# ZhangT-tech/MoCA-Video

Hardware: AMD Instinct MI355X
Metric: denoising UNet-steps/sec @16x320x512 fp16 (higher is better)
Workload: dtype f16

## Files before the change

include/moca_hip.h:

```cpp
#ifndef MOCA_HIP_H
#define MOCA_HIP_H

#include <stdint.h>

#ifdef __cplusplus
extern "C" {
#endif

#define MOCA_OK            0
#define MOCA_E_BADARG     -1
#define MOCA_E_LAUNCH     -2
#define MOCA_E_NODEVICE   -3
#define MOCA_E_GRAPH      -4

#define MOCA_A_LINEAR   0
#define MOCA_A_CONV3X3  1
#define MOCA_A_TCONV3   2

#define MOCA_EP_GEGLU   1
#define MOCA_EP_OUT_F32 2
#define MOCA_FORCE_SMALL_TILE 4
#define MOCA_EP_COLSUM 16
#define MOCA_EP_LN     32
#define MOCA_EP_GELU    8
// ... 44 lines not shown
    float       tattn_scale;
    const void* prefetch;
    int32_t     up_phase;
    int32_t     reserved4_;
    const void* a2;
    int32_t     lda2;
    int32_t     k1;
    int32_t     gstat_cpg;
    int32_t     gstat_coff;
    int32_t     wgroup_rows;
    int32_t     wgroup_stride;
} moca_gemm_params;

int moca_gemm_f16(const moca_gemm_params* p, void* stream);
int moca_gemm_colsum_rows(const moca_gemm_params* p);
int moca_gemm_ln_ok(const moca_gemm_params* p);
int moca_gemm_rowsum_cols(const moca_gemm_params* p);
int moca_gemm_lnfold_ok(const moca_gemm_params* p);
int moca_gemm_tattn_ok(const moca_gemm_params* p);
int moca_gemm_wgroup_ok(const moca_gemm_params* p);
int moca_gemm_cat_ok(const moca_gemm_params* p);
#define MOCA_ROUTE_SMALL64   1
#define MOCA_ROUTE_SMALL128  2
#define MOCA_ROUTE_GLDS128   3
#define MOCA_ROUTE_GLDS160   4
#define MOCA_ROUTE_G4        5
#define MOCA_ROUTE_W80       6
#define MOCA_ROUTE_W80W      7
#define MOCA_ROUTE_SQ256     8
#define MOCA_ROUTE_G4P       9
#define MOCA_ROUTE_SQP       10
#define MOCA_ROUTE_TATTN     11
#define MOCA_ROUTE_WS        12
int moca_gemm_route(const moca_gemm_params* p);
int moca_gemm_splitk_groupnorm_ok(const moca_gemm_params* p, int32_t HW, int32_t frames_per_stat);
int moca_gemm_splitk_groupnorm_f16(const moca_gemm_params* p, void* y, const float* gamma, const float* beta, int32_t HW,
                                   int32_t frames_per_stat, float eps, int32_t silu, int32_t write_x, void* stream);
int64_t moca_gemm_splitk_ws_bytes(int32_t M, int32_t N, int32_t splits);

int moca_groupnorm_nhwc_f16(const void* x, void* y, const float* gamma, const float* beta,
                            int32_t F, int32_t HW, int32_t C, int32_t frames_per_stat,
                            float eps, int32_t silu, float* ws, void* stream);
int64_t moca_groupnorm_ws_bytes(int32_t F, int32_t HW, int32_t C);
int moca_groupnorm_colsum_f16(const void* x, void* y, const float* gamma, const float* beta, const float* colsum,
                              int32_t tile_rows, int32_t F, int32_t HW, int32_t C, int32_t frames_per_stat,
                              float eps, int32_t silu, float* ws, void* stream);

int moca_groupnorm_fold_weights_f16(const void* w, const float* bias, const float* gamma, const float* beta, const int64_t* gstat,
                                    void* wg, float* bg, int32_t n_sg, int32_t N, int32_t K, int32_t ldw, int64_t count, float eps,
                                    void* stream);

int moca_groupnorm_gstat_f16(const void* x, void* y, const float* gamma, const float* beta, const int64_t* gstat,
                             int32_t F, int32_t HW, int32_t C, int32_t frames_per_stat,
                             float eps, int32_t silu, void* stream);
int moca_concat_channels_gstat_f16(const void* a, const void* b, void* out, int32_t F, int32_t HW, int32_t C1, int32_t C2,
                                   int32_t frames_per_stat, int64_t* gstat, void* stream);
int moca_groupnorm_gstat_cat_f16(const void* a, const void* b, void* y, const float* gamma, const float* beta,
                                 const int64_t* gstat_cat, const int64_t* gstat_b, int32_t Fb, int32_t F, int32_t HW, int32_t C1,
                                 int32_t C2, int32_t frames_per_stat, float eps, int32_t silu, void* stream);
int moca_gstat_accum_f16(const void* x, int32_t F, int32_t HW, int32_t C, int32_t frames_per_stat, int32_t cpg, int32_t coff,
                         int64_t* gstat, void* stream);
int moca_memset_zero(void* ptr, int64_t bytes, void* stream);

int moca_layernorm_f16(const void* x, void* y, const float* gamma, const float* beta,
                       int32_t M, int32_t C, float eps, void* stream);

// ... 117 lines not shown
int moca_base_ddim_step_f32(moca_fifo_state* state, float* x, const float* eps_c, const float* eps_u, const float* noise,
                            float* pred_x0, const float* coef, int32_t S, float cfg_scale, int32_t use_scale, int64_t n, void* stream);
int moca_mask_frame_sums_f32(const float* mask, float* sums, int32_t frames, int32_t HW, void* stream);

int moca_freq_mix_3d_f32(const float* x, const float* noise, const float* lpf, float* out,
                         int32_t C, int32_t T, int32_t H, int32_t W, float* ws, void* stream);
int64_t moca_freq_mix_ws_bytes(int32_t C, int32_t T, int32_t H, int32_t W);
int moca_freq_filter_f32(float* lpf, int32_t T, int32_t H, int32_t W, int32_t type, int32_t n,
                         double d_s, double d_t, void* stream);

int moca_graph_begin(void* stream);
int moca_graph_end(void* stream, void** graph_exec_out);
int moca_graph_launch(void* graph_exec, void* stream);
int moca_graph_destroy(void* graph_exec);
int moca_stream_create(void** stream_out);
int moca_stream_destroy(void* stream);
int moca_stream_sync(void* stream);
int moca_event_create(void** ev_out);
int moca_event_record(void* ev, void* stream);
int moca_event_elapsed_ms(void* ev_start, void* ev_stop, float* ms_out);
int moca_event_destroy(void* ev);

#define MOCA_TUNE_GEMM_W80   0
#define MOCA_TUNE_GEMM_G4    1
#define MOCA_TUNE_GEMM_SQ256 2
#define MOCA_TUNE_GEMM_WIDE  3
#define MOCA_TUNE_GN_SLAB    4
#define MOCA_TUNE_GEMM_G4P   5
#define MOCA_TUNE_GEMM_MF32  6
#define MOCA_TUNE_GEMM_SQP   7
#define MOCA_TUNE_SQP_WALK   8
#define MOCA_TUNE_SLAB_F16   9
#define MOCA_TUNE_GEMM_WS    10
#define MOCA_TUNE_COUNT      11
int moca_set_tuning(int32_t knob, int32_t value);
int moca_debug_clock_sampler(void* buf, int32_t blocks, int32_t nsamples, const int32_t* stop, void* stream);

int moca_device_info(char* name, int32_t len, int32_t* cu_count);
const char* moca_version(void);

#ifdef __cplusplus
}
#endif
#endif
```

moca_video_amd/csrc/common.h:

```cpp
#pragma once
#include <hip/hip_runtime.h>
#include <stdint.h>
#include "../../include/moca_hip.h"

typedef _Float16 half_t;
typedef _Float16 half2v __attribute__((ext_vector_type(2)));
typedef _Float16 half4v __attribute__((ext_vector_type(4)));
typedef _Float16 half8v __attribute__((ext_vector_type(8)));
typedef float    f32x4  __attribute__((ext_vector_type(4)));
typedef float    f32x16 __attribute__((ext_vector_type(16)));

#define MOCA_WAVE 64

#define MOCA_CHECK_LAUNCH()                                  \
    do {                                                     \
        hipError_t e__ = hipGetLastError();                  \
        if (e__ != hipSuccess) return MOCA_E_LAUNCH;         \
    } while (0)

static inline hipStream_t moca_stream(void* s) { return reinterpret_cast<hipStream_t>(s); }

int moca_tuning_get(int knob);

bool moca_gemm_ws_ok(const moca_gemm_params& p);
int moca_gemm_ws_launch(const moca_gemm_params& p, hipStream_t st);

__device__ __forceinline__ float moca_silu(float x) {
    return x * __builtin_amdgcn_rcpf(1.0f + __builtin_amdgcn_exp2f(x * -1.4426950408889634f));
}
typedef float f32x2 __attribute__((ext_vector_type(2)));
__device__ __forceinline__ float moca_erf(float x) {
    const float ax = fabsf(x);
    const float t = __builtin_amdgcn_rcpf(1.0f + 0.3275911f * ax);
    float y = 1.061405429f;
    y = y * t - 1.453152027f;
    y = y * t + 1.421413741f;
    y = y * t - 0.284496736f;
    y = y * t + 0.254829592f;
    y = 1.0f - y * t * __builtin_amdgcn_exp2f(ax * ax * -1.4426950408889634f);
    return copysignf(y, x);
}
__device__ __forceinline__ float moca_gelu(float x) { return 0.5f * x * (1.0f + moca_erf(x * 0.70710678118654752f)); }

__device__ __forceinline__ f32x2 moca_erf2(f32x2 x) {
    const f32x2 ax = {fabsf(x[0]), fabsf(x[1])};
    const f32x2 d = ax * 0.3275911f + 1.0f;
    const f32x2 t = {__builtin_amdgcn_rcpf(d[0]), __builtin_amdgcn_rcpf(d[1])};
    f32x2 y = t * 1.061405429f - 1.453152027f;
    y = y * t + 1.421413741f;
    y = y * t - 0.284496736f;
    y = y * t + 0.254829592f;
    const f32x2 a2 = ax * ax * -1.4426950408889634f;
    const f32x2 e = {__builtin_amdgcn_exp2f(a2[0]), __builtin_amdgcn_exp2f(a2[1])};
    y = 1.0f - y * t * e;
    return f32x2{copysignf(y[0], x[0]), copysignf(y[1], x[1])};
}
#ifdef MOCA_GELU_OLD
__device__ __forceinline__ f32x2 moca_geglu2(f32x2 v, f32x2 g) {
// ... 70 lines not shown
```

moca_video_amd/csrc/gemm.hip:

```cpp
#include "gemm_launch.h"

namespace {

template <int BN, int AMODE>
__global__ __launch_bounds__(256, 2) void gemm_f16_kernel(const moca_gemm_params p) {
    constexpr int NT = BN / 64;
    constexpr int B_SLOTS = BN / 32;
    constexpr int A_BYTES = BM * ROW_BYTES;
    constexpr int B_BYTES = BN * ROW_BYTES;

    extern __shared__ __attribute__((aligned(16))) char smem[];
    char* sA = smem;
    char* sB = smem + 2 * A_BYTES;

    const int tid = threadIdx.x, lane = tid & 63, wave = tid >> 6;
    const int wave_m = wave >> 1, wave_n = wave & 1;

    const int tiles_m = (p.M + BM - 1) / BM;
    const int tiles_n = p.N / BN;
    const int nblk = tiles_m * tiles_n * p.splits;
    int logical;
    remap_block<BN>(nblk, logical);
    const int split = logical % p.splits;
    const int tile = logical / p.splits;
// ... 389 lines not shown
            const int c0 = ccol[i] - g * cpg;
            half8v r;
#pragma unroll
            for (int j = 0; j < 8; ++j) {
                float a = (float)v[i][j] * s_sc[c0 + j] + s_sh[c0 + j];
                if (silu) a = moca_silu(a);
                r[j] = (half_t)a;
            }
            *reinterpret_cast<half8v*>(y + (int64_t)mrow[i] * N + ccol[i]) = r;
        }
}

template <int BN, int AMODE>
int launch_gemm(const moca_gemm_params& p, hipStream_t st) {
    const int tiles_m = (p.M + BM - 1) / BM, tiles_n = p.N / BN;
    const int nblk = tiles_m * tiles_n * p.splits;
    constexpr int lds_pipe = 2 * (BM + BN) * ROW_BYTES;
    constexpr int lds_epi = BM * BN * 4;
    constexpr int lds = lds_pipe > lds_epi ? lds_pipe : lds_epi;
    if (!dyn_lds_once<&gemm_f16_kernel<BN, AMODE>>(lds)) return MOCA_E_LAUNCH;
    hipLaunchKernelGGL((gemm_f16_kernel<BN, AMODE>), dim3(nblk), dim3(256), lds, st, p);
    MOCA_CHECK_LAUNCH();
    return MOCA_OK;
}
int launch_gemm_small(int bn, const moca_gemm_params& p, hipStream_t st) {
    if (bn == 128) return with_gather(p, [&](auto am, auto) { return launch_gemm<128, decltype(am)::value>(p, st); });
    return with_gather(p, [&](auto am, auto) { return launch_gemm<64, decltype(am)::value>(p, st); });
}

enum Route : int {
    R_NONE = 0,
    R_SMALL64 = MOCA_ROUTE_SMALL64, R_SMALL128 = MOCA_ROUTE_SMALL128, R_GLDS128 = MOCA_ROUTE_GLDS128, R_GLDS160 = MOCA_ROUTE_GLDS160,
    R_G4 = MOCA_ROUTE_G4, R_W80 = MOCA_ROUTE_W80, R_W80W = MOCA_ROUTE_W80W, R_SQ256 = MOCA_ROUTE_SQ256, R_G4P = MOCA_ROUTE_G4P,
    R_SQP = MOCA_ROUTE_SQP, R_TATTN = MOCA_ROUTE_TATTN, R_WS = MOCA_ROUTE_WS,
};

void normalise_splits(moca_gemm_params& p) {
    if (p.splits < 1) p.splits = 1;
    if (p.splits > (p.K + BK - 1) / BK) p.splits = (p.K + BK - 1) / BK;
    if (p.splits > 1) {
        const int nkt = (p.K + BK - 1) / BK, kts = (nkt + p.splits - 1) / p.splits;
        p.splits = (nkt + kts - 1) / kts;
    }
}

inline int64_t a_span_bytes(const moca_gemm_params& p) {
    if (p.a_mode == MOCA_A_LINEAR) return ((int64_t)p.M * p.lda + 64) * 2;
    if (p.a_mode == MOCA_A_CONV3X3) return ((int64_t)(p.M / (p.outH * p.outW)) * p.inH * p.inW * p.C + 64) * 2;
    return ((int64_t)p.M * p.C + 64) * 2;
}
inline bool buffer_addressable(const moca_gemm_params& p) {
    if (p.a2 && ((int64_t)p.M * p.lda2 + 64) * 2 >= (1ll << 31)) return false;
    return a_span_bytes(p) < (1ll << 31) && (int64_t)p.N * p.ldw * 2 < (1ll << 31);
}

bool persistent_ok(const moca_gemm_params& p, int BN, int blocks) {
    if (p.a_mode != MOCA_A_LINEAR || p.splits != 1 || p.N % BN || p.K % 64 || !buffer_addressable(p)) return false;
    if (p.flags & ~(MOCA_EP_GEGLU | MOCA_EP_LNFOLD)) return false;
    if ((p.flags & MOCA_EP_GEGLU) && (p.residual || p.rowadd)) return false;
    return ((p.M + 255) / 256) * (p.N / BN) >= blocks;
}

Route route_of(const moca_gemm_params& p) {
    if (p.flags & MOCA_EP_TATTN) return R_TATTN;
    const int ws_mode = moca_tuning_get(MOCA_TUNE_GEMM_WS);
    if (ws_mode && moca_gemm_ws_ok(p) && (ws_mode == 2 || p.residual || p.M >= (1 << 17))) return R_WS;
    if (!p.a2 && p.wgroup_rows <= 0) {
        const int sqp_mode = moca_tuning_get(MOCA_TUNE_GEMM_SQP), g4p_mode = moca_tuning_get(MOCA_TUNE_GEMM_G4P);
        if (sqp_mode && persistent_ok(p, 256, SQP_BLOCKS) && (sqp_mode == 2 || (p.flags & MOCA_EP_GEGLU))) return R_SQP;
        if (g4p_mode && persistent_ok(p, 128, G4P_BLOCKS) && (g4p_mode == 2 || (p.flags & MOCA_EP_GEGLU))) return R_G4P;
    }
    const int w80_mode = moca_tuning_get(MOCA_TUNE_GEMM_W80);
    const int tiles320 = ((p.M + 319) / 320) * (p.N / 160);
    if (w80_mode && p.N % 160 == 0 && !(p.flags & (MOCA_EP_GEGLU | MOCA_EP_OUT_F32 | MOCA_FORCE_SMALL_TILE)) && p.M > 160 &&
        (tiles320 * p.splits >= 200 || w80_mode == 2) && fast_gather(p) && buffer_addressable(p)) {
        if (p.flags & MOCA_EP_LN) return R_W80W;
        const int wide_mode = moca_tuning_get(MOCA_TUNE_GEMM_WIDE);
        if (wide_mode == 0 || p.N % 320) return R_W80;
        return (p.a_mode == MOCA_A_LINEAR || wide_mode == 2) ? R_W80W : R_W80;
    }
    const int g4_mode = moca_tuning_get(MOCA_TUNE_GEMM_G4);
    const bool use_g4 = !(p.flags & MOCA_EP_OUT_F32) &&
                        (g4_mode == 2 || (g4_mode == 1 && (p.flags & MOCA_EP_GEGLU) && p.K <= 640 && p.M < (1 << 17)));
    const int sq256_mode = moca_tuning_get(MOCA_TUNE_GEMM_SQ256);
    if (sq256_mode && p.a_mode == MOCA_A_LINEAR && p.N % 256 == 0 && p.N >= 2560 && p.M >= 512 && fast_gather(p) && buffer_addressable(p) &&
        !(p.flags & (MOCA_EP_OUT_F32 | MOCA_FORCE_SMALL_TILE)) && ((p.M + 255) / 256) * (p.N / 256) * p.splits >= 200 &&
        (sq256_mode == 2 || !use_g4)) return R_SQ256;
    const int big_bn = (p.N % 128 == 0) ? 128 : (p.N % 160 == 0 ? 160 : 0);
    if (big_bn != 0 && p.M > 128 && !(p.flags & MOCA_FORCE_SMALL_TILE)) {
        if (big_bn == 128) return use_g4 ? R_G4 : R_GLDS128;
        return R_GLDS160;
    }
    return p.N % 128 == 0 ? R_SMALL128 : R_SMALL64;
}

constexpr int CAN_SPLITK = 1 << 16, CAN_A2 = 1 << 17, CAN_WGROUP = 1 << 18, CAN_UP_PHASE = 1 << 19;
constexpr int EP_STATS = MOCA_EP_COLSUM | MOCA_EP_GSTAT;
struct RouteInfo { int tm, tn, can; };
RouteInfo route_info(Route r) {
    constexpr int GLDS = MOCA_EP_GEGLU | MOCA_EP_OUT_F32 | EP_STATS | MOCA_EP_ROWSUM | MOCA_EP_LNFOLD | CAN_SPLITK | CAN_UP_PHASE;
    constexpr int W80 = EP_STATS | MOCA_EP_ROWSUM | MOCA_EP_LNFOLD | CAN_SPLITK | CAN_UP_PHASE | CAN_A2 | CAN_WGROUP;
    switch (r) {
        case R_SMALL64: return {BM, 64, MOCA_EP_OUT_F32 | MOCA_EP_GELU | CAN_SPLITK};
        case R_SMALL128: return {BM, 128, MOCA_EP_GEGLU | MOCA_EP_OUT_F32 | MOCA_EP_GELU | CAN_SPLITK};
        case R_GLDS128: return {256, 128, GLDS};
        case R_GLDS160: return {256, 160, GLDS};
        case R_G4: return {256, 128, MOCA_EP_GEGLU | MOCA_EP_LNFOLD | CAN_SPLITK | CAN_UP_PHASE};
        case R_W80: return {320, 160, W80};
        case R_W80W: return {160, 320, W80 | MOCA_EP_LN};
        case R_SQ256: return {256, 256, MOCA_EP_GEGLU | MOCA_EP_LNFOLD | CAN_SPLITK};
        case R_G4P: return {256, 128, MOCA_EP_GEGLU | MOCA_EP_LNFOLD};
        case R_SQP: return {256, 256, MOCA_EP_GEGLU | MOCA_EP_LNFOLD};
        case R_TATTN: return {320, 192, MOCA_EP_TATTN | MOCA_EP_LNFOLD};
        case R_WS: return {32, 80, MOCA_EP_ROWSUM | MOCA_EP_GSTAT | CAN_WGROUP};
        case R_NONE: break;
    }
    return {0, 0, 0};
}

bool route_can(Route r, const moca_gemm_params& p) {
    const RouteInfo ri = route_info(r);
    const int f = p.flags & ~(MOCA_FORCE_SMALL_TILE | MOCA_EP_SLABS);
    const int wants = f | (p.splits > 1 ? CAN_SPLITK : 0) | (p.a2 ? CAN_A2 : 0) | (p.wgroup_rows ? CAN_WGROUP : 0) | (p.up_phase ? CAN_UP_PHASE : 0);
    if (r == R_NONE || (wants & ~ri.can) || p.wgroup_rows < 0) return false;
    if (r == R_WS) return true;
    const bool linear1 = p.a_mode == MOCA_A_LINEAR && p.splits == 1;
    if (r == R_TATTN) {
        if (!linear1 || !fast_gather(p) || !buffer_addressable(p) || p.residual || p.rowadd || (p.flags & MOCA_FORCE_SMALL_TILE)) return false;
        if (p.N % 192 || p.T != 16 || p.HW <= 0 || p.HW % 20 || p.M % (16 * p.HW)) return false;
        if (p.ldo % 4 || p.ldo < p.N / 3) return false;
        return p.tattn_causal == 0 || (p.tattn_causal == 1 && p.tattn_scale > 0.f);
    }
    if ((f & EP_STATS) && (p.splits != 1 || (f & (MOCA_EP_GEGLU | MOCA_EP_OUT_F32)))) return false;
    if ((f & MOCA_EP_ROWSUM) && (p.splits != 1 || (f & (MOCA_EP_GEGLU | MOCA_EP_OUT_F32 | EP_STATS | MOCA_EP_LN | MOCA_EP_GELU)))) return false;
    if ((f & MOCA_EP_LN) && !(linear1 && p.N == 320 && !(f & EP_STATS))) return false;
    if ((f & MOCA_EP_LNFOLD) && !(linear1 && !(f & (MOCA_EP_OUT_F32 | EP_STATS | MOCA_EP_LN | MOCA_EP_ROWSUM | MOCA_EP_GELU)) &&
                                  !((r == R_GLDS128 || r == R_GLDS160) && (f & MOCA_EP_GEGLU)))) return false;
    if ((f & MOCA_EP_GELU) && (f & MOCA_EP_GEGLU)) return false;
    if (p.a2) {
        if (!linear1 || (f & ~(EP_STATS | MOCA_EP_ROWSUM))) return false;
        if (p.k1 <= 0 || p.k1 >= p.K || p.k1 % 64 || (p.K - p.k1) % 64 || p.lda % 8 || p.lda2 % 8 || p.lda < p.k1 || p.lda2 < p.K - p.k1) return false;
    }
    if (p.wgroup_rows) {
        if (!linear1 || p.a2 || p.wgroup_stride < p.N * p.ldw || (f & ~(EP_STATS | MOCA_EP_ROWSUM | MOCA_EP_LN))) return false;
        if (p.M % p.wgroup_rows || p.wgroup_rows % ri.tm) return false;
        if ((int64_t)(p.M / p.wgroup_rows) * p.wgroup_stride * 2 >= (1ll << 31)) return false;
    }
    if (p.up_phase && (p.splits != 1 || p.M <= 160 || !fast_gather(p) || p.residual || p.rowadd || (f & ~MOCA_EP_GSTAT) ||
                       (p.N % 128 && p.N % 160))) return false;
    return true;
}

Route checked_route(const moca_gemm_params& p) {
    const Route r = route_of(p);
    return route_can(r, p) ? r : R_NONE;
}

Route query_route(const moca_gemm_params* pp, int flag, moca_gemm_params& p) {
// ... 44 lines not shown
            if (p.up && (p.stride != 1 || p.outH != 2 * p.inH || p.outW != 2 * p.inW)) return R_NONE;
            if (!p.up && p.stride == 1 && (p.outH != p.inH || p.outW != p.inW)) return R_NONE;
            if (p.stride == 2 && (p.outH != (p.inH - 1) / 2 + 1 || p.outW != (p.inW - 1) / 2 + 1)) return R_NONE;
            if (p.M % (p.outH * p.outW)) return R_NONE;
            break;
        case MOCA_A_TCONV3:
            if (p.C % 8 || p.K != 3 * p.C || p.T <= 0 || p.HW <= 0 || p.M % (p.T * p.HW)) return R_NONE;
            break;
        default:
            return R_NONE;
    }
    if (p.a2 && p.a_mode != MOCA_A_LINEAR) return R_NONE;
    if (p.gstat_cpg < 0 || p.gstat_coff < 0 || ((p.gstat_cpg || p.gstat_coff) && !(p.flags & MOCA_EP_GSTAT))) return R_NONE;
    if (p.tattn_causal && !(p.flags & MOCA_EP_TATTN)) return R_NONE;
    const Route r = checked_route(p);
    if (r == R_NONE) return R_NONE;
    if ((p.flags & MOCA_EP_COLSUM) && !p.colsum) return R_NONE;
    if ((p.flags & MOCA_EP_LN) && !(p.ln_gamma && p.ln_beta && p.ln_out && p.ld_ln % 8 == 0)) return R_NONE;
    if ((p.flags & MOCA_EP_ROWSUM) && !p.rowsum) return R_NONE;
    if ((p.flags & MOCA_EP_LNFOLD) && !(p.lnf_part && p.lnf_wsum && p.lnf_nparts >= 1)) return R_NONE;
    if ((p.flags & MOCA_EP_GSTAT) &&
        !(p.gstat && !(p.flags & MOCA_EP_COLSUM) && p.gstat_rows > 0 && p.gstat_rows % route_info(r).tm == 0 && p.M % p.gstat_rows == 0 &&
          (p.gstat_cpg > 0 ? (p.gstat_coff + p.N - 1) / p.gstat_cpg < 32 : (p.N % 32 == 0 && p.gstat_coff == 0)))) return R_NONE;
    p.reserved4_ = 0;
    if ((int64_t)p.M * (geglu ? p.N / 2 : p.N) * 2 >= (128ll << 20)) p.reserved4_ |= 1;
    if (slab_f16(r, p)) p.reserved4_ |= 4;
    return r;
}

int launch_route(Route r, const moca_gemm_params& p, hipStream_t st) {
    switch (r) {
        case R_TATTN: return moca_gemm_w80s_launch(3, p, st);
        case R_WS: return moca_gemm_ws_launch(p, st);
        case R_SQP: return moca_gemm_sqp_launch(p, st);
        case R_G4P: return moca_gemm_g4p_launch(p, st);
        case R_W80: return moca_gemm_w80s_launch(0, p, st);
        case R_W80W: return moca_gemm_w80s_launch(1, p, st);
        case R_SQ256: return moca_gemm_w80s_launch(2, p, st);
        case R_G4: return moca_gemm_g4_launch(p, st);
        case R_GLDS128: return moca_gemm_glds_launch(128, p, st);
        case R_GLDS160: return moca_gemm_glds_launch(160, p, st);
        case R_SMALL128: return launch_gemm_small(128, p, st);
        case R_SMALL64: return launch_gemm_small(64, p, st);
        case R_NONE: break;
    }
    return MOCA_E_BADARG;
}

}

#ifdef MOCA_STAMPS
extern "C" int moca_debug_stamps(unsigned long long* host_out, int n_blocks) {
    if (n_blocks > STAMP_BLOCKS) n_blocks = STAMP_BLOCKS;
    return hipMemcpyFromSymbol(host_out, HIP_SYMBOL(g_stamps), (size_t)n_blocks * STAMP_SLOTS * 8) == hipSuccess ? 0 : -2;
}
#endif

extern "C" int moca_gemm_route(const moca_gemm_params* pp) {
    moca_gemm_params p;
    return prepare(pp, p);
}

extern "C" int moca_gemm_colsum_rows(const moca_gemm_params* pp) {
    moca_gemm_params p;
    return route_info(query_route(pp, (pp && (pp->flags & MOCA_EP_GSTAT)) ? 0 : MOCA_EP_COLSUM, p)).tm;
}
// ... 32 lines not shown
    moca_gemm_params p = *pp;
    if (p.M <= 0 || p.N <= 0 || p.K <= 0 || p.N % 64 || p.K % 8 || !p.splitk_ws || (write_x && !p.out)) return MOCA_E_BADARG;
    if (p.ldo % 8 || (p.residual && p.ldr % 8) || (p.rowadd && (p.ld_rowadd % 8 || p.rowadd_div <= 0))) return MOCA_E_BADARG;
    normalise_splits(p);
    if (!splitk_gn_ok(p, HW, frames_per_stat)) return MOCA_E_BADARG;
    p.reserved4_ = slab_f16(route_of(p), p) ? 4 : 0;
    const int cpg = p.N / 32, R = HW * frames_per_stat;
    const int nchunks = R * (cpg / 8);
    const int cpt = (nchunks + 1023) / 1024;
    int thr = ((nchunks + cpt - 1) / cpt + 63) / 64 * 64;
    if (thr < (cpg + 63) / 64 * 64) thr = (cpg + 63) / 64 * 64;
    const int n_slabs = (p.M / R) * 32;
    const double inv_count = 1.0 / ((double)R * cpg);
    hipStream_t st = moca_stream(stream);
    half_t* yo = reinterpret_cast<half_t*>(y);
#define MOCA_SKGN(CPT) hipLaunchKernelGGL(splitk_gn_kernel<CPT>, dim3(n_slabs), dim3(thr), 0, st, p, yo, gamma, beta, R, cpg, inv_count, eps, silu, write_x)
    if (cpt == 1) MOCA_SKGN(1); else if (cpt == 2) MOCA_SKGN(2); else if (cpt == 3) MOCA_SKGN(3); else MOCA_SKGN(4);
#undef MOCA_SKGN
    MOCA_CHECK_LAUNCH();
    return MOCA_OK;
}

extern "C" int64_t moca_gemm_splitk_ws_bytes(int32_t M, int32_t N, int32_t splits) {
    return splits > 1 ? (int64_t)splits * M * N * 4 : 0;
}

extern "C" int moca_gemm_f16(const moca_gemm_params* pp, void* stream) {
    moca_gemm_params p;
    const Route r = prepare(pp, p);
    if (r == R_NONE) return MOCA_E_BADARG;
    hipStream_t st = moca_stream(stream);
    const int rc = launch_route(r, p, st);
    if (rc != MOCA_OK) return rc;
    if (p.splits > 1 && !(p.flags & MOCA_EP_SLABS)) {
        const int out_n = (p.flags & MOCA_EP_GEGLU) ? p.N / 2 : p.N;
        const int64_t total = (int64_t)p.M * (out_n / 8);
        int blocks = (int)((total + 255) / 256);
        if (blocks > 2048) blocks = 2048;
        hipLaunchKernelGGL(splitk_reduce_kernel, dim3(blocks), dim3(256), 0, st, p);
        MOCA_CHECK_LAUNCH();
    }
    return MOCA_OK;
}

#ifdef MOCA_DIAG_NAME
extern "C" const char* moca_version(void) { return "moca_hip 0.1 (gfx950) DIAG:" MOCA_DIAG_NAME; }
#else
extern "C" const char* moca_version(void) { return "moca_hip 0.1 (gfx950)"; }
#endif
```

moca_video_amd/csrc/gemm_launch.h:

```cpp
#ifndef MOCA_GEMM_LAUNCH_H
#define MOCA_GEMM_LAUNCH_H
#include "gemm_device.h"

int moca_gemm_glds_launch(int bn, const moca_gemm_params& p, hipStream_t st);
int moca_gemm_g4_launch(const moca_gemm_params& p, hipStream_t st);
int moca_gemm_w80s_launch(int shape, const moca_gemm_params& p, hipStream_t st);
int moca_gemm_g4p_launch(const moca_gemm_params& p, hipStream_t st);
int moca_gemm_sqp_launch(const moca_gemm_params& p, hipStream_t st);

namespace {

constexpr int G4P_BLOCKS = 512;
constexpr int SQP_BLOCKS = 256;

static int choose_xcd_n(const moca_gemm_params& p, int tiles_m, int tiles_n, int BN) {
    if (p.splits != 1 || p.a_mode != MOCA_A_LINEAR) return 1;
    const double Wtot = (double)p.N * p.K * 2, Atot = (double)p.M * p.K * 2;
    auto cost = [&](int xn) {
        const int xm = 8 / xn;
        const double wsub = (double)(tiles_n / xn) * BN * p.K * 2;
        return (wsub <= 3.6e6 ? xm * Wtot : tiles_m * Wtot) + xn * Atot;
    };
    double best = cost(1);
    int best_xn = 1;
    for (int xn = 2; xn <= 8; xn *= 2) {
        if (tiles_m % (8 / xn) || tiles_n % xn) continue;
        const double c = cost(xn);
        if (c < 0.8 * best) { best = c; best_xn = xn; }
    }
    return best_xn;
}

inline bool fast_gather(const moca_gemm_params& p) {
    return (p.a_mode == MOCA_A_LINEAR) ? (p.K % BK == 0 && p.K <= 8192) : (p.C % BK == 0 && p.C <= 8192);
}
template <typename F>
int with_gather(const moca_gemm_params& p, F f) {
    const bool fast = fast_gather(p);
    if (p.a_mode == MOCA_A_LINEAR) return fast ? f(int_c<MOCA_A_LINEAR>{}, yes_t{}) : f(int_c<MOCA_A_LINEAR>{}, no_t{});
    if (p.a_mode == MOCA_A_CONV3X3) return fast ? f(int_c<MOCA_A_CONV3X3>{}, yes_t{}) : f(int_c<MOCA_A_CONV3X3>{}, no_t{});
    return fast ? f(int_c<MOCA_A_TCONV3>{}, yes_t{}) : f(int_c<MOCA_A_TCONV3>{}, no_t{});
}

template <auto KERNEL>
bool dyn_lds_once(int lds) {
    static bool attr_set = false;
    if (!attr_set) {
        if (hipFuncSetAttribute(reinterpret_cast<const void*>(KERNEL), hipFuncAttributeMaxDynamicSharedMemorySize, lds) != hipSuccess) return false;
        attr_set = true;
    }
    return true;
}

}

#endif
```

moca_video_amd/csrc/runtime.hip:

```cpp
#include "common.h"
#include <string.h>
#include <stdio.h>
#include <stdlib.h>

extern "C" int moca_graph_begin(void* stream) {
    if (hipStreamBeginCapture(moca_stream(stream), hipStreamCaptureModeThreadLocal) != hipSuccess) return MOCA_E_GRAPH;
    return MOCA_OK;
}

extern "C" int moca_graph_end(void* stream, void** graph_exec_out) {
    if (!graph_exec_out) return MOCA_E_BADARG;
    hipGraph_t g = nullptr;
    if (hipStreamEndCapture(moca_stream(stream), &g) != hipSuccess || !g) return MOCA_E_GRAPH;
    hipGraphExec_t ge = nullptr;
    hipError_t e = hipGraphInstantiate(&ge, g, nullptr, nullptr, 0);
    (void)hipGraphDestroy(g);
    if (e != hipSuccess || !ge) return MOCA_E_GRAPH;
    *graph_exec_out = reinterpret_cast<void*>(ge);
    return MOCA_OK;
}

extern "C" int moca_graph_launch(void* graph_exec, void* stream) {
    if (!graph_exec) return MOCA_E_BADARG;
    if (hipGraphLaunch(reinterpret_cast<hipGraphExec_t>(graph_exec), moca_stream(stream)) != hipSuccess) return MOCA_E_GRAPH;
// ... 65 lines not shown
    const int64_t n16 = bytes / 16;
    int blocks = (int)((n16 + 255) / 256);
    if (blocks < 1) blocks = 1;
    if (blocks > 1024) blocks = 1024;
    hipLaunchKernelGGL(zero_kernel, dim3(blocks), dim3(256), 0, moca_stream(stream), reinterpret_cast<uint4*>(ptr), n16,
                       reinterpret_cast<unsigned char*>(ptr) + n16 * 16, (int)(bytes - n16 * 16));
    MOCA_CHECK_LAUNCH();
    return MOCA_OK;
}

__global__ __launch_bounds__(64) void clock_sampler_kernel(unsigned long long* __restrict__ buf, int nsamples, const volatile int* stop) {
#if defined(__HIP_DEVICE_COMPILE__)
    if (threadIdx.x) return;
    unsigned long long* b = buf + (size_t)blockIdx.x * nsamples * 2;
    for (int i = 0; i < nsamples; ++i) {
        unsigned long long t, r;
        asm volatile("s_memtime %0\n\ts_memrealtime %1\n\ts_waitcnt lgkmcnt(0)" : "=s"(t), "=s"(r)::"memory");
        b[2 * i] = t;
        b[2 * i + 1] = r;
        if (stop && *stop) break;
        __builtin_amdgcn_s_sleep(127);
        __builtin_amdgcn_s_sleep(127);
    }
#endif
}
extern "C" int moca_debug_clock_sampler(void* buf, int32_t blocks, int32_t nsamples, const int32_t* stop, void* stream) {
    if (!buf || blocks < 1 || blocks > 64 || nsamples < 1 || nsamples > (1 << 20)) return MOCA_E_BADARG;
    hipLaunchKernelGGL(clock_sampler_kernel, dim3(blocks), dim3(64), 0, moca_stream(stream), reinterpret_cast<unsigned long long*>(buf), nsamples,
                       reinterpret_cast<const volatile int*>(stop));
    MOCA_CHECK_LAUNCH();
    return MOCA_OK;
}

static int g_tuning[MOCA_TUNE_COUNT] = {1, 1, 1, 1, 1, 1, 0, 1, 0, 0, 1};
int moca_tuning_get(int knob) { return (knob >= 0 && knob < MOCA_TUNE_COUNT) ? g_tuning[knob] : 0; }
extern "C" int moca_set_tuning(int32_t knob, int32_t value) {
    if (knob < 0 || knob >= MOCA_TUNE_COUNT || value < 0 || value > 2) return MOCA_E_BADARG;
    const int old = g_tuning[knob];
    g_tuning[knob] = value;
    return old;
}
```

moca_video_amd/lib.py:

```python
from __future__ import annotations

import ctypes as C
import os

import torch

_HERE = os.path.dirname(os.path.abspath(__file__))
LIB_PATH = os.environ.get("MOCA_HIP_LIB") or os.path.join(_HERE, "libmoca_hip.so")

MOCA_A_LINEAR, MOCA_A_CONV3X3, MOCA_A_TCONV3 = 0, 1, 2
MOCA_EP_GEGLU, MOCA_EP_OUT_F32, MOCA_FORCE_SMALL_TILE, MOCA_EP_GELU, MOCA_EP_COLSUM, MOCA_EP_LN = 1, 2, 4, 8, 16, 32
MOCA_EP_ROWSUM, MOCA_EP_LNFOLD, MOCA_EP_GSTAT, MOCA_EP_TATTN, MOCA_EP_SLABS = 64, 128, 256, 512, 1024
MOCA_TUNE_GEMM_W80, MOCA_TUNE_GEMM_G4, MOCA_TUNE_GEMM_SQ256, MOCA_TUNE_GEMM_WIDE, MOCA_TUNE_GN_SLAB, MOCA_TUNE_GEMM_G4P, MOCA_TUNE_GEMM_MF32, MOCA_TUNE_GEMM_SQP, MOCA_TUNE_SQP_WALK = 0, 1, 2, 3, 4, 5, 6, 7, 8
MOCA_TUNE_SLAB_F16 = 9
MOCA_TUNE_GEMM_WS = 10
(MOCA_ROUTE_SMALL64, MOCA_ROUTE_SMALL128, MOCA_ROUTE_GLDS128, MOCA_ROUTE_GLDS160, MOCA_ROUTE_G4, MOCA_ROUTE_W80, MOCA_ROUTE_W80W,
 MOCA_ROUTE_SQ256, MOCA_ROUTE_G4P, MOCA_ROUTE_SQP, MOCA_ROUTE_TATTN, MOCA_ROUTE_WS) = range(1, 13)

_ERR = {0: "ok", -1: "bad argument (shape/alignment contract)", -2: "HIP launch/runtime error",
        -3: "no gfx950 device", -4: "graph capture/replay failed"}


class MocaHipError(RuntimeError):
    pass


class GemmParams(C.Structure):
    _fields_ = [
        ("a", C.c_void_p), ("w", C.c_void_p), ("out", C.c_void_p), ("bias", C.c_void_p),
        ("rowadd", C.c_void_p), ("residual", C.c_void_p), ("splitk_ws", C.c_void_p),
        ("M", C.c_int32), ("N", C.c_int32), ("K", C.c_int32),
        ("lda", C.c_int32), ("ldw", C.c_int32), ("ldo", C.c_int32), ("ldr", C.c_int32), ("ld_rowadd", C.c_int32),
        ("rowadd_div", C.c_int32), ("a_mode", C.c_int32), ("C", C.c_int32),
        ("inH", C.c_int32), ("inW", C.c_int32), ("outH", C.c_int32), ("outW", C.c_int32),
        ("stride", C.c_int32), ("up", C.c_int32), ("T", C.c_int32), ("HW", C.c_int32),
        ("flags", C.c_int32), ("splits", C.c_int32), ("nopad_lo", C.c_int32), ("prefetch_kib", C.c_int32),
        ("tattn_causal", C.c_int32),
        ("colsum", C.c_void_p), ("ln_gamma", C.c_void_p), ("ln_beta", C.c_void_p), ("ln_out", C.c_void_p),
        ("ld_ln", C.c_int32), ("ln_eps", C.c_float),
        ("rowsum", C.c_void_p), ("lnf_part", C.c_void_p), ("lnf_wsum", C.c_void_p),
        ("lnf_nparts", C.c_int32), ("reserved2_", C.c_int32),
        ("gstat", C.c_void_p), ("gstat_rows", C.c_int32), ("tattn_scale", C.c_float),
        ("prefetch", C.c_void_p), ("up_phase", C.c_int32), ("reserved4_", C.c_int32),
        ("a2", C.c_void_p), ("lda2", C.c_int32), ("k1", C.c_int32), ("gstat_cpg", C.c_int32), ("gstat_coff", C.c_int32),
        ("wgroup_rows", C.c_int32), ("wgroup_stride", C.c_int32),
    ]


class FifoState(C.Structure):
    _fields_ = [("head", C.c_int32), ("iter", C.c_int32), ("seed_lo", C.c_uint32), ("seed_hi", C.c_uint32),
# ... 152 lines not shown
```

Measured before the change: 61.94.

## Add whole-K GEMM route replacing split-K with in-register split accumulation

Adds a new GEMM kernel (64x128 tile, 4-slot LDS pipeline with buffer-to-LDS loads) that walks the full K range in one block instead of launching split-K partials plus a separate reduction pass. It accumulates per-split segments in registers so rounding matches the split-K order, and applies bias, rowadd and residual directly in the epilogue. It is enabled by default for a hand-picked list of shapes that currently use splits 2 or 4. The aim is to remove the split-K workspace traffic and reduction kernel launch, at the cost of fewer blocks and less parallelism per GEMM.

```diff
diff --git a/include/moca_hip.h b/include/moca_hip.h
--- a/include/moca_hip.h
+++ b/include/moca_hip.h
@@ -100,6 +100,7 @@
 #define MOCA_ROUTE_SQP       10
 #define MOCA_ROUTE_TATTN     11
 #define MOCA_ROUTE_WS        12
+#define MOCA_ROUTE_WK        13
 int moca_gemm_route(const moca_gemm_params* p);
 int moca_gemm_splitk_groupnorm_ok(const moca_gemm_params* p, int32_t HW, int32_t frames_per_stat);
 int moca_gemm_splitk_groupnorm_f16(const moca_gemm_params* p, void* y, const float* gamma, const float* beta, int32_t HW,
@@ -283,7 +284,8 @@
 #define MOCA_TUNE_SQP_WALK   8
 #define MOCA_TUNE_SLAB_F16   9
 #define MOCA_TUNE_GEMM_WS    10
-#define MOCA_TUNE_COUNT      11
+#define MOCA_TUNE_GEMM_WK    11
+#define MOCA_TUNE_COUNT      12
 int moca_set_tuning(int32_t knob, int32_t value);
 int moca_debug_clock_sampler(void* buf, int32_t blocks, int32_t nsamples, const int32_t* stop, void* stream);
 
diff --git a/moca_video_amd/csrc/common.h b/moca_video_amd/csrc/common.h
--- a/moca_video_amd/csrc/common.h
+++ b/moca_video_amd/csrc/common.h
@@ -24,6 +24,8 @@
 
 bool moca_gemm_ws_ok(const moca_gemm_params& p);
 int moca_gemm_ws_launch(const moca_gemm_params& p, hipStream_t st);
+bool moca_gemm_wk_ok(const moca_gemm_params& p);
+int moca_gemm_wk_launch(const moca_gemm_params& p, hipStream_t st);
 
 __device__ __forceinline__ float moca_silu(float x) {
     return x * __builtin_amdgcn_rcpf(1.0f + __builtin_amdgcn_exp2f(x * -1.4426950408889634f));
diff --git a/moca_video_amd/csrc/gemm.hip b/moca_video_amd/csrc/gemm.hip
--- a/moca_video_amd/csrc/gemm.hip
+++ b/moca_video_amd/csrc/gemm.hip
@@ -445,7 +445,7 @@
     R_NONE = 0,
     R_SMALL64 = MOCA_ROUTE_SMALL64, R_SMALL128 = MOCA_ROUTE_SMALL128, R_GLDS128 = MOCA_ROUTE_GLDS128, R_GLDS160 = MOCA_ROUTE_GLDS160,
     R_G4 = MOCA_ROUTE_G4, R_W80 = MOCA_ROUTE_W80, R_W80W = MOCA_ROUTE_W80W, R_SQ256 = MOCA_ROUTE_SQ256, R_G4P = MOCA_ROUTE_G4P,
-    R_SQP = MOCA_ROUTE_SQP, R_TATTN = MOCA_ROUTE_TATTN, R_WS = MOCA_ROUTE_WS,
+    R_SQP = MOCA_ROUTE_SQP, R_TATTN = MOCA_ROUTE_TATTN, R_WS = MOCA_ROUTE_WS, R_WK = MOCA_ROUTE_WK,
 };
 
 void normalise_splits(moca_gemm_params& p) {
@@ -457,16 +457,6 @@
     }
 }
 
-inline int64_t a_span_bytes(const moca_gemm_params& p) {
-    if (p.a_mode == MOCA_A_LINEAR) return ((int64_t)p.M * p.lda + 64) * 2;
-    if (p.a_mode == MOCA_A_CONV3X3) return ((int64_t)(p.M / (p.outH * p.outW)) * p.inH * p.inW * p.C + 64) * 2;
-    return ((int64_t)p.M * p.C + 64) * 2;
-}
-inline bool buffer_addressable(const moca_gemm_params& p) {
-    if (p.a2 && ((int64_t)p.M * p.lda2 + 64) * 2 >= (1ll << 31)) return false;
-    return a_span_bytes(p) < (1ll << 31) && (int64_t)p.N * p.ldw * 2 < (1ll << 31);
-}
-
 bool persistent_ok(const moca_gemm_params& p, int BN, int blocks) {
     if (p.a_mode != MOCA_A_LINEAR || p.splits != 1 || p.N % BN || p.K % 64 || !buffer_addressable(p)) return false;
     if (p.flags & ~(MOCA_EP_GEGLU | MOCA_EP_LNFOLD)) return false;
@@ -474,10 +464,20 @@
     return ((p.M + 255) / 256) * (p.N / BN) >= blocks;
 }
 
+bool wk_measured(const moca_gemm_params& p) {
+    if (p.N == 1280 && p.splits == 4) {
+        if (p.M == 1280) return (p.a_mode == MOCA_A_TCONV3 && p.K == 3840) || (p.a_mode == MOCA_A_LINEAR && (p.K == 2560 || p.K == 5120));
+        if (p.M == 640) return p.a_mode == MOCA_A_LINEAR && p.K == 2560;
+    }
+    return p.a_mode == MOCA_A_CONV3X3 && p.M == 2560 && p.N == 640 && p.K == 5760 && p.splits == 2;
+}
+
 Route route_of(const moca_gemm_params& p) {
     if (p.flags & MOCA_EP_TATTN) return R_TATTN;
     const int ws_mode = moca_tuning_get(MOCA_TUNE_GEMM_WS);
     if (ws_mode && moca_gemm_ws_ok(p) && (ws_mode == 2 || p.residual || p.M >= (1 << 17))) return R_WS;
+    const int wk_mode = moca_tuning_get(MOCA_TUNE_GEMM_WK);
+    if (wk_mode && moca_gemm_wk_ok(p) && (wk_mode == 2 || wk_measured(p))) return R_WK;
     if (!p.a2 && p.wgroup_rows <= 0) {
         const int sqp_mode = moca_tuning_get(MOCA_TUNE_GEMM_SQP), g4p_mode = moca_tuning_get(MOCA_TUNE_GEMM_G4P);
         if (sqp_mode && persistent_ok(p, 256, SQP_BLOCKS) && (sqp_mode == 2 || (p.flags & MOCA_EP_GEGLU))) return R_SQP;
@@ -526,6 +526,7 @@
         case R_SQP: return {256, 256, MOCA_EP_GEGLU | MOCA_EP_LNFOLD};
         case R_TATTN: return {320, 192, MOCA_EP_TATTN | MOCA_EP_LNFOLD};
         case R_WS: return {32, 80, MOCA_EP_ROWSUM | MOCA_EP_GSTAT | CAN_WGROUP};
+        case R_WK: return {64, 128, CAN_SPLITK};
         case R_NONE: break;
     }
     return {0, 0, 0};
@@ -536,7 +537,7 @@
     const int f = p.flags & ~(MOCA_FORCE_SMALL_TILE | MOCA_EP_SLABS);
     const int wants = f | (p.splits > 1 ? CAN_SPLITK : 0) | (p.a2 ? CAN_A2 : 0) | (p.wgroup_rows ? CAN_WGROUP : 0) | (p.up_phase ? CAN_UP_PHASE : 0);
     if (r == R_NONE || (wants & ~ri.can) || p.wgroup_rows < 0) return false;
-    if (r == R_WS) return true;
+    if (r == R_WS || r == R_WK) return true;
     const bool linear1 = p.a_mode == MOCA_A_LINEAR && p.splits == 1;
     if (r == R_TATTN) {
         if (!linear1 || !fast_gather(p) || !buffer_addressable(p) || p.residual || p.rowadd || (p.flags & MOCA_FORCE_SMALL_TILE)) return false;
@@ -647,6 +648,7 @@
     switch (r) {
         case R_TATTN: return moca_gemm_w80s_launch(3, p, st);
         case R_WS: return moca_gemm_ws_launch(p, st);
+        case R_WK: return moca_gemm_wk_launch(p, st);
         case R_SQP: return moca_gemm_sqp_launch(p, st);
         case R_G4P: return moca_gemm_g4p_launch(p, st);
         case R_W80: return moca_gemm_w80s_launch(0, p, st);
@@ -745,7 +747,7 @@
     hipStream_t st = moca_stream(stream);
     const int rc = launch_route(r, p, st);
     if (rc != MOCA_OK) return rc;
-    if (p.splits > 1 && !(p.flags & MOCA_EP_SLABS)) {
+    if (p.splits > 1 && !(p.flags & MOCA_EP_SLABS) && r != R_WK) {
         const int out_n = (p.flags & MOCA_EP_GEGLU) ? p.N / 2 : p.N;
         const int64_t total = (int64_t)p.M * (out_n / 8);
         int blocks = (int)((total + 255) / 256);
diff --git a/moca_video_amd/csrc/gemm_launch.h b/moca_video_amd/csrc/gemm_launch.h
--- a/moca_video_amd/csrc/gemm_launch.h
+++ b/moca_video_amd/csrc/gemm_launch.h
@@ -34,6 +34,15 @@
 inline bool fast_gather(const moca_gemm_params& p) {
     return (p.a_mode == MOCA_A_LINEAR) ? (p.K % BK == 0 && p.K <= 8192) : (p.C % BK == 0 && p.C <= 8192);
 }
+inline int64_t a_span_bytes(const moca_gemm_params& p) {
+    if (p.a_mode == MOCA_A_LINEAR) return ((int64_t)p.M * p.lda + 64) * 2;
+    if (p.a_mode == MOCA_A_CONV3X3) return ((int64_t)(p.M / (p.outH * p.outW)) * p.inH * p.inW * p.C + 64) * 2;
+    return ((int64_t)p.M * p.C + 64) * 2;
+}
+inline bool buffer_addressable(const moca_gemm_params& p) {
+    if (p.a2 && ((int64_t)p.M * p.lda2 + 64) * 2 >= (1ll << 31)) return false;
+    return a_span_bytes(p) < (1ll << 31) && (int64_t)p.N * p.ldw * 2 < (1ll << 31);
+}
 template <typename F>
 int with_gather(const moca_gemm_params& p, F f) {
     const bool fast = fast_gather(p);
diff --git a/moca_video_amd/csrc/gemm_wk.hip b/moca_video_amd/csrc/gemm_wk.hip
--- /dev/null
+++ b/moca_video_amd/csrc/gemm_wk.hip
@@ -0,0 +1,235 @@
+#include "gemm_launch.h"
+
+namespace {
+
+constexpr int WK_TM = 64, WK_BN = 128;
+[[maybe_unused]] constexpr int WK_SLOTS = 4, WK_AHEAD = WK_SLOTS - 1;
+[[maybe_unused]] constexpr int WK_A_BYTES = WK_TM * ROW_BYTES;
+constexpr int WK_STAGE = (WK_TM + WK_BN) * ROW_BYTES;
+[[maybe_unused]] constexpr int WK_PPW = 6;
+constexpr int WK_LDS = WK_SLOTS * WK_STAGE;
+constexpr int WK_MIN_K = 1024;
+
+template <int AMODE>
+__global__ __launch_bounds__(256, 2) void gemm_wk_kernel(const moca_gemm_params p) {
+#if defined(__HIP_DEVICE_COMPILE__)
+    constexpr int NT = 4;
+    extern __shared__ __attribute__((aligned(16))) char smem[];
+
+    const int tid = threadIdx.x, lane = tid & 63;
+    const int wave = __builtin_amdgcn_readfirstlane(tid >> 6);
+    const int wave_m = wave >> 1, wave_n = wave & 1;
+
+    const int tiles_m = (p.M + WK_TM - 1) / WK_TM, tiles_n = p.N / WK_BN;
+    int tile_m, tile_n;
+    if ((p.reserved4_ >> 8) > 1) {
+        remap_tile_2d(tiles_m, tiles_n, p.reserved4_ >> 8, tile_m, tile_n);
+    } else {
+        int logical;
+        remap_block<WK_BN>(tiles_m * tiles_n, logical);
+        tile_m = logical / tiles_n; tile_n = logical - tile_m * tiles_n;
+    }
+    const int m0 = tile_m * WK_TM, n0 = tile_n * WK_BN;
+    const int nk = p.K / BK;
+    const int kts = (nk + p.splits - 1) / p.splits;
+
+    const int lrow = lane >> 3, pch = lane & 7;
+    const int lch = pch ^ ((wave * 4 + (lrow >> 1)) & 7);
+    BGather<AMODE, 2, BK> ga(p, lch, 0, 0);
+#pragma unroll
+    for (int g = 0; g < 2; ++g) ga.init_row(g, m0 + (g * 4 + wave) * 8 + lrow);
+    unsigned w_off[4];
+#pragma unroll
+    for (int g = 0; g < 4; ++g) w_off[g] = (unsigned)((((int64_t)(n0 + (g * 4 + wave) * 8 + lrow)) * p.ldw + lch * 8) * 2);
+    const __amdgpu_buffer_rsrc_t rsrc_a = __builtin_amdgcn_make_buffer_rsrc(const_cast<void*>(p.a), 0, OOB_OFF, 0x00020000);
+    const __amdgpu_buffer_rsrc_t rsrc_w = __builtin_amdgcn_make_buffer_rsrc(const_cast<void*>(p.w), 0, OOB_OFF, 0x00020000);
+    const int tiles_per_tap = AMODE == MOCA_A_LINEAR ? (1 << 30) : p.C / BK;
+    int s_tap = 0, s_tin = 0, s_kt = 0;
+    ga.set_tap(0);
+
+    auto dma_piece = [&](int slot, int j) {
+        const bool live = s_kt < nk;
+        const lds_ptr sa = (lds_ptr)smem + slot * WK_STAGE;
+        if (j < 2) __builtin_amdgcn_raw_ptr_buffer_load_lds(rsrc_a, sa + (j * 4 + wave) * 1024, 16, live ? ga.a_off[j] : OOB_OFF,
+                                                            live ? (unsigned)(s_tin * BK * 2) : 0u, 0, 0);
+        else __builtin_amdgcn_raw_ptr_buffer_load_lds(rsrc_w, sa + WK_A_BYTES + ((j - 2) * 4 + wave) * 1024, 16, live ? w_off[j - 2] : OOB_OFF,
+                                                      live ? (unsigned)(s_kt * BK * 2) : 0u, 0, 0);
+    };
+    auto stream_next = [&]() {
+        ++s_kt;
+        if (++s_tin == tiles_per_tap) { s_tin = 0; ga.set_tap(++s_tap); }
+    };
+
+    f32x4 acc[2][NT], tot[2][NT];
+    const int fr = lane & 15, fg = lane >> 4;
+#pragma unroll
+    for (int nt = 0; nt < NT; ++nt) {
+        const f32x4 bv = ld4_or_zero(p.bias, n0 + wave_n * 64 + nt * 16 + 4 * fg);
+#pragma unroll
+        for (int mt = 0; mt < 2; ++mt) { acc[mt][nt] = f32x4{0.f, 0.f, 0.f, 0.f}; tot[mt][nt] = bv; }
+    }
+    int a_row_b[2], a_swz[2], b_row_b[NT], b_swz[NT];
+#pragma unroll
+    for (int mt = 0; mt < 2; ++mt) {
+        const int row = wave_m * 32 + mt * 16 + fr;
+        a_row_b[mt] = row * ROW_BYTES;
+        a_swz[mt] = (row >> 1) & 7;
+    }
+#pragma unroll
+    for (int nt = 0; nt < NT; ++nt) {
+        const int row = wave_n * 64 + nt * 16 + fr;
+        b_row_b[nt] = WK_A_BYTES + row * ROW_BYTES;
+        b_swz[nt] = (row >> 1) & 7;
+    }
+    half8v af0[2], bf0[NT], af1[2], bf1[NT];
+    auto read_one = [&](const char* st, int ks, int r, half8v (&af)[2], half8v (&bf)[NT]) {
+        const int ch = ks * 4 + fg;
+        if (r < 2) af[r] = *reinterpret_cast<const half8v*>(st + a_row_b[r] + ((ch ^ a_swz[r]) << 4));
+        else bf[r - 2] = *reinterpret_cast<const half8v*>(st + b_row_b[r - 2] + ((ch ^ b_swz[r - 2]) << 4));
+    };
+    constexpr int NMMA = 2 * NT, NRD = 2 + NT;
+
+#pragma unroll
+    for (int s = 0; s < WK_AHEAD; ++s) {
+#pragma unroll
+        for (int j = 0; j < WK_PPW; ++j) dma_piece(s, j);
+        stream_next();
+    }
+    asm volatile("s_waitcnt vmcnt(%0)" ::"n"((WK_AHEAD - 1) * WK_PPW) : "memory");
+    __builtin_amdgcn_s_barrier();
+#pragma unroll
+    for (int r = 0; r < NRD; ++r) read_one(smem, 0, r, af0, bf0);
+
+    int s_cur = 0, s_far = WK_AHEAD;
+    int seg = 0;
+    for (int i = 0; i < nk; ++i) {
+        const char* cur = smem + s_cur * WK_STAGE;
+#pragma unroll
+        for (int j = 0; j < NMMA; ++j) {
+            const int mt = j / NT, nt = j % NT;
+            acc[mt][nt] = __builtin_amdgcn_mfma_f32_16x16x32_f16(bf0[nt], af0[mt], acc[mt][nt], 0, 0, 0);
+            if (j < NRD) {
+                read_one(cur, 1, j, af1, bf1);
+                dma_piece(s_far, j);
+            }
+            __builtin_amdgcn_sched_barrier(0);
+        }
+        stream_next();
+        asm volatile("s_waitcnt vmcnt(%0) lgkmcnt(0)" ::"n"((WK_AHEAD - 1) * WK_PPW) : "memory");
+        __builtin_amdgcn_s_barrier();
+        s_cur = s_cur + 1 == WK_SLOTS ? 0 : s_cur + 1;
+        s_far = s_far + 1 == WK_SLOTS ? 0 : s_far + 1;
+        const char* nxt = smem + s_cur * WK_STAGE;
+#pragma unroll
+        for (int j = 0; j < NMMA; ++j) {
+            const int mt = j / NT, nt = j % NT;
+            acc[mt][nt] = __builtin_amdgcn_mfma_f32_16x16x32_f16(bf1[nt], af1[mt], acc[mt][nt], 0, 0, 0);
+            if (j < NRD) read_one(nxt, 0, j, af0, bf0);
+            __builtin_amdgcn_sched_barrier(0);
+        }
+        if (++seg == kts) {
+            seg = 0;
+#pragma unroll
+            for (int mt = 0; mt < 2; ++mt)
+#pragma unroll
+                for (int nt = 0; nt < NT; ++nt) { tot[mt][nt] += acc[mt][nt]; acc[mt][nt] = f32x4{0.f, 0.f, 0.f, 0.f}; }
+        }
+    }
+    if (seg != 0) {
+#pragma unroll
+        for (int mt = 0; mt < 2; ++mt)
+#pragma unroll
+            for (int nt = 0; nt < NT; ++nt) tot[mt][nt] += acc[mt][nt];
+    }
+    asm volatile("s_waitcnt vmcnt(0) lgkmcnt(0)" ::: "memory");
+    __syncthreads();
+
+    float* sC = reinterpret_cast<float*>(smem);
+    constexpr int PF = WK_BN + 4;
+    const bool staged16 = p.splits == 1 && p.M > 128;
+#pragma unroll
+    for (int mt = 0; mt < 2; ++mt)
+#pragma unroll
+        for (int nt = 0; nt < NT; ++nt) {
+            f32x4 v = tot[mt][nt];
+            if (staged16) v = __builtin_convertvector(__builtin_convertvector(v, half4v), f32x4);
+            *reinterpret_cast<f32x4*>(sC + (wave_m * 32 + mt * 16 + fr) * PF + wave_n * 64 + nt * 16 + 4 * fg) = v;
+        }
+    __syncthreads();
+    const half_t* __restrict__ rowadd = reinterpret_cast<const half_t*>(p.rowadd);
+    const half_t* __restrict__ resid = reinterpret_cast<const half_t*>(p.residual);
+    constexpr int U = WK_TM * (WK_BN / 8) / 256;
+    const half8v zero8 = {0, 0, 0, 0, 0, 0, 0, 0};
+    half8v ea[U], er[U];
+#pragma unroll
+    for (int u = 0; u < U; ++u) {
+        const int idx = tid + u * 256, row = idx >> 4, col = n0 + (idx & 15) * 8, m = m0 + row;
+        ea[u] = zero8; er[u] = zero8;
+        if (m < p.M) {
+            if (rowadd) ea[u] = *reinterpret_cast<const half8v*>(rowadd + (int64_t)(m / p.rowadd_div) * p.ld_rowadd + col);
+            if (resid) er[u] = *reinterpret_cast<const half8v*>(resid + (int64_t)m * p.ldr + col);
+        }
+    }
+#pragma unroll
+    for (int u = 0; u < U; ++u) {
+        const int idx = tid + u * 256, row = idx >> 4, ch = idx & 15, m = m0 + row;
+        if (m >= p.M) continue;
+        const f32x4 c0 = *reinterpret_cast<const f32x4*>(sC + row * PF + ch * 8), c1 = *reinterpret_cast<const f32x4*>(sC + row * PF + ch * 8 + 4);
+        float v[8] = {c0[0], c0[1], c0[2], c0[3], c1[0], c1[1], c1[2], c1[3]};
+        half8v h;
+#pragma unroll
+        for (int j = 0; j < 8; ++j) {
+            if (rowadd) v[j] += (float)ea[u][j];
+            if (resid) v[j] += (float)er[u][j];
+            h[j] = (half_t)v[j];
+        }
+        *reinterpret_cast<half8v*>(reinterpret_cast<half_t*>(p.out) + (int64_t)m * p.ldo + n0 + ch * 8) = h;
+    }
+#endif
+}
+
+int wk_xcd_n(const moca_gemm_params& p, int tiles_m, int tiles_n) {
+    const double W = (double)p.N * p.K * 2, A = (double)p.M * (p.a_mode == MOCA_A_LINEAR ? p.K : p.C) * 2;
+    const double share = (double)(tiles_m * tiles_n / 8 + 1) / tiles_n;
+    double best = 8 * W * (share < 1.0 ? share : 1.0) + A * (share < 0.125 ? 8.0 : share < 1.0 ? 1.0 / share : 1.0);
+    int best_xn = 0;
+    for (int xn = 1; xn <= 8; xn *= 2) {
+        const int xm = 8 / xn;
+        if (tiles_m % xm || tiles_n % xn) continue;
+        const double c = W * xm + A * xn;
+        if (c < 0.9 * best) { best = c; best_xn = xn; }
+    }
+    return best_xn;
+}
+
+template <int AMODE>
+int wk_launch1(const moca_gemm_params& pp, hipStream_t st) {
+    moca_gemm_params p = pp;
+    const int tiles_m = (p.M + WK_TM - 1) / WK_TM, tiles_n = p.N / WK_BN;
+    const int nblk = tiles_m * tiles_n;
+    p.reserved4_ = (p.reserved4_ & 0xff) | (wk_xcd_n(p, tiles_m, tiles_n) << 8);
+    if (!dyn_lds_once<&gemm_wk_kernel<AMODE>>(WK_LDS)) return MOCA_E_LAUNCH;
+    hipLaunchKernelGGL((gemm_wk_kernel<AMODE>), dim3(nblk), dim3(256), WK_LDS, st, p);
+    MOCA_CHECK_LAUNCH();
+    return MOCA_OK;
+}
+
+}
+
+bool moca_gemm_wk_ok(const moca_gemm_params& p) {
+    if (p.flags || p.a2 || p.wgroup_rows || p.up_phase || p.prefetch_kib > 0) return false;
+    if (p.a_mode != MOCA_A_LINEAR && p.a_mode != MOCA_A_CONV3X3 && p.a_mode != MOCA_A_TCONV3) return false;
+    if (p.M <= 0 || p.K < WK_MIN_K || p.K % BK || p.N % WK_BN || p.splits < 1) return false;
+    if (!fast_gather(p) || !buffer_addressable(p)) return false;
+    if ((int64_t)((p.M + WK_TM - 1) / WK_TM) * (p.N / WK_BN) >= (1ll << 31)) return false;
+    if ((reinterpret_cast<uintptr_t>(p.a) | reinterpret_cast<uintptr_t>(p.w) | reinterpret_cast<uintptr_t>(p.out) | reinterpret_cast<uintptr_t>(p.bias) |
+         reinterpret_cast<uintptr_t>(p.rowadd) | reinterpret_cast<uintptr_t>(p.residual)) & 15) return false;
+    return true;
+}
+
+int moca_gemm_wk_launch(const moca_gemm_params& p, hipStream_t st) {
+    if (!moca_gemm_wk_ok(p)) return MOCA_E_BADARG;
+    if (p.a_mode == MOCA_A_LINEAR) return wk_launch1<MOCA_A_LINEAR>(p, st);
+    if (p.a_mode == MOCA_A_CONV3X3) return wk_launch1<MOCA_A_CONV3X3>(p, st);
+    return wk_launch1<MOCA_A_TCONV3>(p, st);
+}
diff --git a/moca_video_amd/csrc/runtime.hip b/moca_video_amd/csrc/runtime.hip
--- a/moca_video_amd/csrc/runtime.hip
+++ b/moca_video_amd/csrc/runtime.hip
@@ -121,7 +121,7 @@
     return MOCA_OK;
 }
 
-static int g_tuning[MOCA_TUNE_COUNT] = {1, 1, 1, 1, 1, 1, 0, 1, 0, 0, 1};
+static int g_tuning[MOCA_TUNE_COUNT] = {1, 1, 1, 1, 1, 1, 0, 1, 0, 0, 1, 1};
 int moca_tuning_get(int knob) { return (knob >= 0 && knob < MOCA_TUNE_COUNT) ? g_tuning[knob] : 0; }
 extern "C" int moca_set_tuning(int32_t knob, int32_t value) {
     if (knob < 0 || knob >= MOCA_TUNE_COUNT || value < 0 || value > 2) return MOCA_E_BADARG;
diff --git a/moca_video_amd/lib.py b/moca_video_amd/lib.py
--- a/moca_video_amd/lib.py
+++ b/moca_video_amd/lib.py
@@ -14,8 +14,9 @@
 MOCA_TUNE_GEMM_W80, MOCA_TUNE_GEMM_G4, MOCA_TUNE_GEMM_SQ256, MOCA_TUNE_GEMM_WIDE, MOCA_TUNE_GN_SLAB, MOCA_TUNE_GEMM_G4P, MOCA_TUNE_GEMM_MF32, MOCA_TUNE_GEMM_SQP, MOCA_TUNE_SQP_WALK = 0, 1, 2, 3, 4, 5, 6, 7, 8
 MOCA_TUNE_SLAB_F16 = 9
 MOCA_TUNE_GEMM_WS = 10
+MOCA_TUNE_GEMM_WK = 11
 (MOCA_ROUTE_SMALL64, MOCA_ROUTE_SMALL128, MOCA_ROUTE_GLDS128, MOCA_ROUTE_GLDS160, MOCA_ROUTE_G4, MOCA_ROUTE_W80, MOCA_ROUTE_W80W,
- MOCA_ROUTE_SQ256, MOCA_ROUTE_G4P, MOCA_ROUTE_SQP, MOCA_ROUTE_TATTN, MOCA_ROUTE_WS) = range(1, 13)
+ MOCA_ROUTE_SQ256, MOCA_ROUTE_G4P, MOCA_ROUTE_SQP, MOCA_ROUTE_TATTN, MOCA_ROUTE_WS, MOCA_ROUTE_WK) = range(1, 14)
 
 _ERR = {0: "ok", -1: "bad argument (shape/alignment contract)", -2: "HIP launch/runtime error",
         -3: "no gfx950 device", -4: "graph capture/replay failed"}
```

Measured after the change: 62.17 (median of 6 runs). About the same (+0.4%).
